# facebookresearch/FBTT-Embedding

Measured on AMD Instinct MI355X. Metric: fwd+bwd GFLOPS (true algorithmic: 3 x fwd FLOP / time), TT-EmbeddingBag E=11M D=64 ranks=[32, 32] nnz=10240, higher is better.
Workload: dtype f32

## Files before the change

fbtt-embedding_amd/csrc/ttx_internal.h:

```cpp
#pragma once
#include <hip/hip_runtime.h>
#include <stdint.h>
#include <stdio.h>
#include <string.h>

#include "../../include/ttx.h"
#ifdef TTX_TEST_HOOKS
#include "../../include/ttx_test_hooks.h"
#define TTX_KNOB(type, name, dflt) type name = dflt
#else
#define TTX_KNOB(type, name, dflt) constexpr type name = dflt
#endif

namespace ttx {

constexpr int kWave = 64;

void set_error(const char* fmt, ...);
#define TTX_FAIL(code, ...)     \
  do {                          \
    ttx::set_error(__VA_ARGS__); \
    return (code);              \
  } while (0)
#define TTX_HIP(call)                                                         \
  do {                                                                        \
    hipError_t e__ = (call);                                                  \
    if (e__ != hipSuccess)                                                    \
      TTX_FAIL(TTX_EHIP, "%s failed: %s", #call, hipGetErrorString(e__));     \
  } while (0)

inline size_t align_up(size_t x, size_t a = 256) { return (x + a - 1) / a * a; }

int allow_dynamic_lds(const void* kernel, int bytes);
int device_cus();

struct UDiv {
  unsigned m, sh1, sh2, d;
};

struct TabGeom {
  int p[TTX_MAX_TABLES_MIXED][TTX_MAX_CORES];
  int base[TTX_MAX_TABLES_MIXED][TTX_MAX_CORES];
  long long L[TTX_MAX_TABLES_MIXED][TTX_MAX_CORES];
};

struct Dims {
  int T, num_tables;
  const TabGeom* tab;
  int p[TTX_MAX_CORES], q[TTX_MAX_CORES], r[TTX_MAX_CORES + 1];
  long long L[TTX_MAX_CORES];
  int slice[TTX_MAX_CORES];
  int S[TTX_MAX_CORES];
  int m[TTX_MAX_CORES], k[TTX_MAX_CORES], n[TTX_MAX_CORES];
  int D;
  int idx32;
  UDiv dvL[TTX_MAX_CORES], dvP[TTX_MAX_CORES];
};

int make_dims(const ttx_geom* g, Dims* d);

#ifndef TTX_SEG_THIN
#define TTX_SEG_THIN 256
#endif
#ifndef TTX_HOT_PIVOT
#define TTX_HOT_PIVOT 16
#endif
constexpr int kSegThin = TTX_SEG_THIN;
constexpr int kHotRowsPivot = TTX_HOT_PIVOT;

constexpr int kHdrT4Valid = 20;
struct Plan {
  int* hdr;
  int* sid[TTX_MAX_CORES];
  int* perm[TTX_MAX_CORES];
  int* ipos[TTX_MAX_CORES];
  int* off[TTX_MAX_CORES];
  int* chunk_off;
  int4* chunk_rec;
  int4* lrec;
  int* lrow;
  int* cnt;
  int* scratch[TTX_MAX_CORES][3];
  int max_chunks;
  int MC;
  float* t4m;
  float* t4g;
  int4* t4o;
};

int choose_chunk(const Dims& d, long long nnz);
size_t t4_scratch_floats(const Dims& d);
int max_chunks(const Dims& d, long long nnz, int MC);
size_t plan_bytes(const Dims& d, long long nnz);
Plan carve_plan(const Dims& d, long long nnz, void* base);
int plan_build(const Dims& d, long long nnz, const int64_t* indices,
               const int64_t* tableidx, const int64_t* rowidx, const Plan& P, hipStream_t stream,
               const int* n_dev = nullptr, const int64_t* offsets = nullptr, int bags_per_table = 0);

constexpr int kMaxMulti = 16;
struct ProBatch {
  const int64_t* indices[kMaxMulti];
  const int64_t* offsets[kMaxMulti];
  long long out_stride;
  long long plan_stride;
};
#define TTX_PICK_BATCH(MB, Z, IND, OFF)                                                                   \
  switch (Z) {                                                                                            \
    case 1: IND = MB.indices[1]; OFF = MB.offsets[1]; break;                                              \
    case 2: IND = MB.indices[2]; OFF = MB.offsets[2]; break;                                              \
    case 3: IND = MB.indices[3]; OFF = MB.offsets[3]; break;                                              \
    case 4: IND = MB.indices[4]; OFF = MB.offsets[4]; break;                                              \
    case 5: IND = MB.indices[5]; OFF = MB.offsets[5]; break;                                              \
    case 6: IND = MB.indices[6]; OFF = MB.offsets[6]; break;                                              \
    case 7: IND = MB.indices[7]; OFF = MB.offsets[7]; break;                                              \
    case 8: IND = MB.indices[8]; OFF = MB.offsets[8]; break;                                              \
    case 9: IND = MB.indices[9]; OFF = MB.offsets[9]; break;                                              \
    case 10: IND = MB.indices[10]; OFF = MB.offsets[10]; break;                                           \
    case 11: IND = MB.indices[11]; OFF = MB.offsets[11]; break;                                           \
    case 12: IND = MB.indices[12]; OFF = MB.offsets[12]; break;                                           \
    case 13: IND = MB.indices[13]; OFF = MB.offsets[13]; break;                                           \
    case 14: IND = MB.indices[14]; OFF = MB.offsets[14]; break;                                           \
    case 15: IND = MB.indices[15]; OFF = MB.offsets[15]; break;                                           \
    default: break;                                                                                       \
  }
bool plan_batches_ok(const Dims& d, long long nnz);
int plan_build_batches(const Dims& d, int nbatch, long long nnz, const int* n_dev, const int64_t* indices,
                       const int64_t* tableidx, const int64_t* rowidx, void* plans, size_t plan_stride,
                       hipStream_t stream);

long long* debug_stamps();

int fill_iota64(int64_t* dst, long long n, hipStream_t stream);

struct DedupMap {
  int* nu;
  int64_t* uidx;
  int64_t* utab;
  int64_t* iota;
  int* uid;
  int* occ;
  int* occ_off;
};
constexpr int kDedupMaxN = 16384;
__host__ __device__ inline int64_t* dedup_tstart(const DedupMap& M) { return (int64_t*)((char*)M.nu + 64); }
int dedup_max_tables();
bool plan_groups_tables(const Dims& d, long long N);
bool dedup_supported(const Dims& d, long long nnz);
size_t dedup_bytes(long long nnz);
DedupMap carve_dedup(long long nnz, void* base);
int dedup_build(const Dims& d, long long nnz, const int64_t* indices, const int64_t* tableidx, const DedupMap& M,
                hipStream_t stream);
void dedup_key_buffers(const DedupMap& M, long long nnz, int64_t** keys, int64_t** vals);
int dedup_build_from_keys(long long nnz, unsigned long long all, const DedupMap& M, hipStream_t stream);
size_t gsum_scratch_bytes(int D, long long nnz);
int gsum_launch(const DedupMap& M, long long nnz, int B, int D, const int64_t* rowidx, const int64_t* tableidx, const float* psw,
                const float* d_output, float* Gu, void* scratch, hipStream_t st, long long skip_key = -1);

size_t sort_pairs_ws_bytes(int64_t n);
int sort_pairs_desc(int64_t n, const int64_t* keys_in, const int64_t* vals_in, char* ws, int64_t** keys_sorted,
                    int64_t** vals_sorted, hipStream_t st, int passes);

size_t populate_sort_ws_bytes(int64_t H);
int populate_sort_mark(int64_t H, int64_t* hashtbl, int64_t* cache_freq, int32_t* cache_state, int64_t cache_size,
                       int keep_state, char* ws, int64_t** sorted_keys, hipStream_t st);

void prof_begin(int which, hipStream_t s);
void prof_end(int which, hipStream_t s);
struct ProfScope {
  int w;
  hipStream_t s;
  ProfScope(int which, hipStream_t st) : w(which), s(st) { prof_begin(w, s); }
// ... 91 lines not shown
```

fbtt-embedding_amd/csrc/ttx_plan.hip:

```cpp
#include <stdlib.h>

#include <type_traits>

#include "ttx_internal.h"

namespace ttx {

constexpr int kPlanThreads = 1024;
constexpr int kPlanWaves = kPlanThreads / kWave;

#ifdef TTX_TEST_HOOKS
static int g_plan_route = 0;
#define TTX_PLAN_ROUTE(id) (g_plan_route = (id))
#else
#define TTX_PLAN_ROUTE(id) ((void)0)
#endif

int max_chunks(const Dims& d, long long nnz, int MC) {
  if (MC <= 0) MC = 1;
  long long a = nnz < d.S[1] ? nnz : d.S[1];
  long long v = a + nnz / MC + 1;
  return (int)v;
}

static size_t r64(size_t k) { return (k + 63) / 64 * 64; }

constexpr int kMaxGroupsHost = 32;
static size_t cnt_ints(const Dims& d, long long nnz) {
  return (size_t)d.T * (256 * ((nnz + 255) / 256 + 1) + 2048 * (kMaxGroupsHost + 2));
}

static size_t plan_ints(const Dims& d, long long nnz, int MC) {
  size_t n = r64(64);
  for (int t = 0; t < d.T; ++t) n += r64(nnz) * 6 + r64((size_t)d.S[t] + 1);
  n += r64((size_t)d.S[1] + 1);
  n += r64((size_t)max_chunks(d, nnz, MC) * 4);
  n += r64((size_t)nnz * 4);
  n += r64((size_t)nnz);
  n += r64(cnt_ints(d, nnz));
  if (const size_t tf = t4_scratch_floats(d)) n += 2 * r64((size_t)nnz * tf) + r64((size_t)nnz * 4);
  return n;
}

size_t plan_bytes(const Dims& d, long long nnz) {
  return align_up(plan_ints(d, nnz, choose_chunk(d, nnz)) * sizeof(int));
}

Plan carve_plan(const Dims& d, long long nnz, void* base) {
  Plan P;
  memset(&P, 0, sizeof(P));
  P.MC = choose_chunk(d, nnz);
  P.max_chunks = max_chunks(d, nnz, P.MC);
  int* cur = (int*)base;
  auto take = [&](size_t k) { int* r = cur; cur += r64(k); return r; };
  P.hdr = take(64);
  P.chunk_rec = (int4*)take((size_t)P.max_chunks * 4);
  P.lrec = (int4*)take((size_t)nnz * 4);
  P.lrow = take(nnz);
  P.cnt = take(cnt_ints(d, nnz));
  for (int t = 0; t < d.T; ++t) {
    P.sid[t] = take(nnz);
    P.perm[t] = take(nnz);
    P.ipos[t] = take(nnz);
    P.off[t] = take((size_t)d.S[t] + 1);
    for (int i = 0; i < 3; ++i) P.scratch[t][i] = take(nnz);
  }
  P.chunk_off = take((size_t)d.S[1] + 1);
  if (const size_t tf = t4_scratch_floats(d)) {
    P.t4m = (float*)take((size_t)nnz * tf);
    P.t4g = (float*)take((size_t)nnz * tf);
    P.t4o = (int4*)take((size_t)nnz * 4);
  }
  return P;
}

__device__ __forceinline__ int block_excl_scan(int v, int* wtot, int* total) {
  const int lane = lane_id();
  const int w = threadIdx.x / kWave;
  int inc = wave_incl_scan(v);
  if (lane == kWave - 1) wtot[w] = inc;
  __syncthreads();
  if (threadIdx.x == 0) {
    int run = 0;
    for (int i = 0; i < kPlanWaves; ++i) { int c = wtot[i]; wtot[i] = run; run += c; }
    wtot[kPlanWaves] = run;
  }
  __syncthreads();
  int res = wtot[w] + inc - v;
  *total = wtot[kPlanWaves];
  __syncthreads();
  return res;
}

struct CoreDec {
  UDiv dl, dp;
  long long L;
  int p, first, idx32;
};
__device__ __forceinline__ CoreDec core_dec(const Dims& d, int t) {
  CoreDec c;
  c.dl = d.dvL[t];
  c.dp = d.dvP[t];
  c.L = d.L[t];
  c.p = d.p[t];
  c.first = (t == 0);
  c.idx32 = d.idx32;
  return c;
}
__device__ __forceinline__ int decode_core(const CoreDec& c, long long idx) {
  if (idx < 0) idx = 0;
  if (c.idx32 && (unsigned long long)idx < (1ull << 32)) {
    const unsigned q = udiv((unsigned)idx, c.dl);
    const unsigned a = c.first ? q : q - udiv(q, c.dp) * c.dp.d;
    return (int)min(a, (unsigned)(c.p - 1));
  }
  long long a = idx / c.L;
  if (!c.first) a = a % c.p;
  if (a >= c.p) a = c.p - 1;
  return (int)a;
}
__device__ __forceinline__ int decode_core(const Dims& d, int t, long long idx) {
  return decode_core(core_dec(d, t), idx);
}
__device__ __forceinline__ int slice_id(const Dims& d, const CoreDec& ct, int t, int tb, long long idx) {
  if (!d.tab) return tb * ct.p + decode_core(ct, idx);
  tb = min(max(tb, 0), d.num_tables - 1);
  const int p = d.tab->p[tb][t];
  const long long L = d.tab->L[tb][t];
  if (idx < 0) idx = 0;
  long long a;
  if ((((unsigned long long)idx | (unsigned long long)L) >> 32) == 0) a = (unsigned)idx / (unsigned)L;
  else a = idx / L;
  if (t > 0) a %= p;
  if (a >= p) a = p - 1;
  return d.tab->base[tb][t] + (int)a;
// ... 192 lines not shown
    if (tid == 0) {
      P.chunk_off[S1] = carry;
      P.hdr[0] = carry;
      P.hdr[1] = MC;
      P.hdr[2] = N;
      P.hdr[3] = rowidx ? 1 : 0;
      P.hdr[kHdrT4Valid] = 0;
      for (int tt = 0; tt < TTX_MAX_CORES; ++tt) P.hdr[8 + tt] = -1;
    }
    PSTAMP(5);
  }
#undef PSTAMP
}

constexpr int kMbThreads = 256;
constexpr int kMbUnits = kMbThreads / kWave;
constexpr int kSB = 4;
constexpr int kMbFuseU = 256;

struct MbArgs {
  int N, U;
  const int* n_dev;
  int unit;
  int* cnt;
};

__device__ __forceinline__ int live_n(int n_host, const int* n_dev) {
  if (!n_dev) return n_host;
  const int v = *n_dev;
  return v < 0 ? 0 : (v < n_host ? v : n_host);
}

struct MbItem { int val, kv; };

__device__ __forceinline__ MbItem mb_load(int i, bool valid, int pass, const Dims& d, int t, const CoreDec& ct,
                                          const int64_t* __restrict__ indices, const int64_t* __restrict__ tableidx,
                                          const int* __restrict__ src, const int* __restrict__ key) {
  MbItem it{0, 0};
  if (!valid) return it;
  if (pass == 0) {
    const int tb = tableidx ? (int)tableidx[i] : 0;
    it.val = i;
    it.kv = slice_id(d, ct, t, tb, indices[i]);
  } else {
    it.val = src[i];
    it.kv = key[it.val];
  }
  return it;
}

__global__ __launch_bounds__(kMbThreads) void mb_count_kernel(
    Dims d, MbArgs A, const int64_t* __restrict__ indices, const int64_t* __restrict__ tableidx) {
  __shared__ int hist[kMbUnits][256];
  const int t = blockIdx.y;
  const int lane = lane_id(), w = threadIdx.x / kWave;
  const int u = blockIdx.x * kMbUnits + w;
  for (int e = lane; e < 256; e += kWave) hist[w][e] = 0;
  const int N = live_n(A.N, A.n_dev);
  const int beg = min(N, u * A.unit), end = min(N, beg + A.unit);
  const CoreDec ct = core_dec(d, t);
  for (int base = beg; base < end; base += kSB * kWave) {
    MbItem it[kSB];
#pragma unroll
    for (int k = 0; k < kSB; ++k) {
      const int i = base + k * kWave + lane;
      it[k] = mb_load(i, i < end, 0, d, t, ct, indices, tableidx, nullptr, nullptr);
    }
#pragma unroll
    for (int k = 0; k < kSB; ++k) {
      const int i = base + k * kWave + lane;
      const bool valid = i < end;
      const unsigned dg = (unsigned)it[k].kv & 255u;
      const unsigned long long peers = wave_match8(dg, valid);
      if (valid && (peers & lanemask_lt()) == 0) hist[w][dg] += __popcll(peers);
    }
  }
  if (u < A.U)
    for (int e = lane; e < 256; e += kWave) A.cnt[((size_t)t * A.U + u) * 256 + e] = hist[w][e];
}

template <typename T>
__device__ __forceinline__ T* shifted(T* p, long long bytes) { return (T*)((char*)p + bytes); }

__device__ __forceinline__ void finish_single_pass(const Dims& d, int t, int dg, int tot, int dbase, int N,
                                                   bool has_row, const Plan& P, int* wt5, long long psh = 0) {
  int* const hdr = (int*)((char*)P.hdr + psh);
  int* const chunk_off = (int*)((char*)P.chunk_off + psh);
  int4* const chunk_rec = (int4*)((char*)P.chunk_rec + psh);
  const int lane = lane_id(), w = threadIdx.x / kWave;
  const int S = d.S[t];
  if (t != 1) {
    const int nhot = __syncthreads_count(dg < S && tot > 2 * kSegThin);
    if (dg == 0) hdr[8 + t] = nhot;
    if (dg <= S) shifted(P.off[t], psh)[dg] = (dg == S) ? N : dbase;
    if (dg == 0 && S == 256) shifted(P.off[t], psh)[256] = N;
    return;
  }
  const int MC = P.MC;
  const int nf = dg < S ? tot / MC : 0;
  const int pr = dg < S ? tot - nf * MC : 0;
  const int np = pr ? 1 : 0;
  const int nhot = __syncthreads_count(nf + np > kHotRowsPivot);
  if (dg == 0) hdr[8 + 1] = nhot;
  const int packed = (nf << 12) | np;
  const int cinc = wave_incl_scan(packed);
  __syncthreads();
  if (lane == kWave - 1 && w < kMbUnits) wt5[w] = cinc;
  __syncthreads();
  int cb = 0, call = 0;
  for (int k = 0; k < kMbUnits; ++k) { const int v = wt5[k]; if (k < w) cb += v; call += v; }
  const int exq = cb + cinc - packed;
  const int fbase = exq >> 12, pbase = exq & 4095;
  const int ftot = call >> 12, ptot = call & 4095;
  const int ctot = ftot + ptot;
  const int ex = fbase + pbase;
  __shared__ int cf_base[257], cf_pos[256], cf_slot[256];
  if (dg < S) {
    chunk_off[dg] = ex;
    cf_base[dg] = fbase;
    cf_pos[dg] = dbase;
    cf_slot[dg] = ex;
    if (np) chunk_rec[ftot + pbase] = make_int4(dg, dbase + nf * MC, pr, ex + nf);
  }
  if (dg == 0) cf_base[S] = ftot;
  __syncthreads();
  for (int c = threadIdx.x; c < ftot; c += blockDim.x) {
    int lo = 0, hi = S;
    while (hi - lo > 1) {
      const int mid = (lo + hi) >> 1;
      if (cf_base[mid] <= c) lo = mid; else hi = mid;
    }
    const int j = c - cf_base[lo];
    chunk_rec[c] = make_int4(lo, cf_pos[lo] + j * MC, MC, cf_slot[lo] + j);
  }
  for (int cc = ctot + dg; cc < P.max_chunks; cc += blockDim.x) chunk_rec[cc] = make_int4(0, 0, 0, 0);
  if (dg == 0) {
    chunk_off[S] = ctot;
    hdr[0] = ctot;
    hdr[1] = MC;
    hdr[2] = N;
    hdr[3] = has_row ? 1 : 0;
    hdr[kHdrT4Valid] = 0;
  }
}

constexpr int kOneUnit = 64;
constexpr int kOneMaxN = 16384;
constexpr int kProMaxBags = 4096;
struct Prologue {
  const int64_t* offsets;
  int nb;
  int64_t* rowidx;
  int64_t* tableidx;
  int H;
  int64_t* hashtbl;
  int64_t* cache_freq;
};
#ifndef TTX_PLAN_XWG
#define TTX_PLAN_XWG 1
#endif
constexpr int kOneThreads = 1024;
constexpr int kOneWaves = kOneThreads / kWave;
template <bool PRO>
__global__ __launch_bounds__(kOneThreads) void mb_single_kernel(
    Dims d, int Nmax, const int* __restrict__ n_dev, const int64_t* __restrict__ indices,
    const int64_t* __restrict__ tableidx, const int64_t* __restrict__ rowidx, Plan P, Prologue pg, ProBatch mb) {
  if (PRO && blockIdx.z > 0) {
    const int z = blockIdx.z;
    TTX_PICK_BATCH(mb, z, indices, pg.offsets)
    pg.rowidx += (long long)z * mb.out_stride;
    pg.tableidx += (long long)z * mb.out_stride;
  }
  if (!PRO && blockIdx.z > 0) {
    const long long sh = (long long)blockIdx.z * mb.out_stride;
    indices += sh;
    if (tableidx) tableidx += sh;
    if (rowidx) rowidx += sh;
    if (n_dev) n_dev += blockIdx.z;
  }
  const long long psh = (long long)blockIdx.z * mb.plan_stride;
  __shared__ int haft[256], hbef[256], hrun[kOneWaves][256];
  const int N = live_n(Nmax, n_dev);
  __shared__ int wt5[kMbUnits + 1];
  __shared__ int offs[PRO ? kProMaxBags + 1 : 1];
  const int t = blockIdx.y, tid = threadIdx.x;
  const int lane = lane_id(), w = tid / kWave;
  const CoreDec ct = core_dec(d, t);
  if (PRO) tableidx = nullptr;
  constexpr int kMaxB = kOneMaxN / kOneThreads;
  const int nbat = (N + kOneThreads - 1) / kOneThreads;
  long long ix[kMaxB];
  int tb[kMaxB];
#pragma unroll
  for (int m = 0; m < kMaxB; ++m) {
    const int i = m * kOneThreads + tid;
    ix[m] = (m < nbat && i < N) ? indices[i] : 0;
    tb[m] = (m < nbat && i < N && tableidx) ? (int)tableidx[i] : 0;
  }
  if (PRO) {
    if (t <= 1)
      for (int e = tid; e <= pg.nb; e += kOneThreads) offs[e] = (int)min(pg.offsets[e], (int64_t)0x7fffffff);
  }
  if (tid < 256) { haft[tid] = 0; hbef[tid] = 0; }
  for (int e = tid; e < kOneWaves * 256; e += kOneThreads) (&hrun[0][0])[e] = 0;
  __syncthreads();
  const int bx = blockIdx.x;
  const int bbeg = bx * (kOneWaves * kOneUnit), bend = min(N, bbeg + kOneWaves * kOneUnit);
  const int i = bbeg + tid;
  const bool valid = i < bend;
  int kv = 0, tbv = 0, row = 0;
  long long idx = 0;
  bool peel_on = true;
#pragma unroll
  for (int m = 0; m < kMaxB; ++m) {
    if (m < nbat) {
      const int im = m * kOneThreads + tid;
// ... 204 lines not shown
      a += len > 0 ? (len + kWideSpan - 1) / kWideSpan : 1;
    }
    gwg[ga.ngroups] = a;
  }
  __syncthreads();
  const int g = blockIdx.x;
  if (g >= gwg[ga.ngroups]) return false;
  int k = 0;
  while (k + 1 < ga.ngroups && gwg[k + 1] <= g) ++k;
  m->k = k;
  m->tb0 = k * ga.gsz;
  m->pos0 = gpos[k];
  m->beg = min(gpos[k + 1], gpos[k] + (g - gwg[k]) * kWideSpan);
  m->end = min(gpos[k + 1], m->beg + kWideSpan);
  m->wg0 = gwg[k];
  m->wg1 = gwg[k + 1];
  return true;
}
__device__ __forceinline__ int slice_base(const Dims& d, const CoreDec& ct, int t, int tb) {
  if (tb >= d.num_tables) return d.S[t];
  return d.tab ? d.tab->base[tb][t] : tb * ct.p;
}

template <int BITS, bool GRP>
__global__ __launch_bounds__(kWideThreads) void mbw_count_kernel(
    Dims d, int Nmax, const int* __restrict__ n_dev, const int64_t* __restrict__ indices,
    const int64_t* __restrict__ tableidx, int* __restrict__ cnt, GrpArgs ga) {
  constexpr int BINS = 1 << BITS;
  __shared__ int hist[BINS];
  __shared__ int gpos[GRP ? kMaxGroups + 1 : 1], gwg[GRP ? kMaxGroups + 1 : 1];
  const int t = blockIdx.y, tid = threadIdx.x;
  for (int e = tid; e < BINS; e += kWideThreads) hist[e] = 0;
  const int N = live_n(Nmax, n_dev);
  const CoreDec ct = core_dec(d, t);
  int beg = blockIdx.x * kWideSpan, end = min(N, beg + kWideSpan), sb = 0;
  if (GRP) {
    GrpMap m;
    if (!grp_map(d, ga, N, gpos, gwg, &m)) return;
    beg = m.beg;
    end = m.end;
    sb = slice_base(d, ct, t, m.tb0);
  } else {
    __syncthreads();
  }
  long long ix[kSB];
  int tb[kSB];
#pragma unroll
  for (int k = 0; k < kSB; ++k) {
    const int i = beg + k * kWideThreads + tid;
    ix[k] = i < end ? indices[i] : 0;
    tb[k] = (i < end && tableidx) ? (int)tableidx[i] : 0;
  }
#pragma unroll
  for (int k = 0; k < kSB; ++k) {
    const int i = beg + k * kWideThreads + tid;
    if (i < end) atomicAdd(&hist[min(max(slice_id(d, ct, t, tb[k], ix[k]) - sb, 0), BINS - 1)], 1);
  }
  __syncthreads();
  int* row = cnt + ((size_t)t * gridDim.x + blockIdx.x) * BINS;
  for (int e = tid; e < BINS; e += kWideThreads) row[e] = hist[e];
}

template <int K>
__device__ __forceinline__ void finish_wide(const Dims& d, int t, const int (&tot)[K], const int (&dbase)[K], int N,
                                            bool has_row, const Plan& P, int* wt) {
  const int tid = threadIdx.x, lane = lane_id(), w = tid / kWave;
  const int S = d.S[t];
  if (t != 1) {
    int nh = 0;
#pragma unroll
    for (int j = 0; j < K; ++j) {
      const int dg = tid * K + j;
      if (dg < S) P.off[t][dg] = dbase[j];
      nh += (dg < S && tot[j] > 2 * kSegThin) ? 1 : 0;
    }
    if (tid == 0) wt[0] = 0;
    __syncthreads();
    if (nh) atomicAdd(&wt[0], nh);
    __syncthreads();
    if (tid == 0) { P.off[t][S] = N; P.hdr[8 + t] = wt[0]; }
    return;
  }
  const int MC = P.MC;
  int nf[K], pr[K], packed[K], psum = 0;
#pragma unroll
  for (int j = 0; j < K; ++j) {
    const int dg = tid * K + j;
    nf[j] = dg < S ? tot[j] / MC : 0;
    pr[j] = dg < S ? tot[j] - nf[j] * MC : 0;
    packed[j] = (nf[j] << 13) | (pr[j] ? 1 : 0);
    psum += packed[j];
  }
  const int cinc = wave_incl_scan(psum);
  __syncthreads();
  if (lane == kWave - 1) wt[w] = cinc;
  __syncthreads();
  int cb = 0, call = 0;
  for (int k = 0; k < kWideWaves; ++k) { const int v = wt[k]; if (k < w) cb += v; call += v; }
  int exq = cb + cinc - psum;
  const int ftot = call >> 13, ptot = call & 8191;
  const int ctot = ftot + ptot;
#pragma unroll
  for (int j = 0; j < K; ++j) {
    const int dg = tid * K + j;
    const int fbase = exq >> 13, pbase = exq & 8191;
    const int ex = fbase + pbase;
    if (dg < S) {
      P.chunk_off[dg] = ex;
      for (int jj = 0; jj < nf[j]; ++jj) P.chunk_rec[fbase + jj] = make_int4(dg, dbase[j] + jj * MC, MC, ex + jj);
      if (pr[j]) P.chunk_rec[ftot + pbase] = make_int4(dg, dbase[j] + nf[j] * MC, pr[j], ex + nf[j]);
    }
    exq += packed[j];
  }
  for (int cc = ctot + tid; cc < P.max_chunks; cc += kWideThreads) P.chunk_rec[cc] = make_int4(0, 0, 0, 0);
  int nh = 0;
#pragma unroll
  for (int j = 0; j < K; ++j) nh += (tid * K + j < S && nf[j] + (pr[j] ? 1 : 0) > kHotRowsPivot) ? 1 : 0;
  __syncthreads();
  if (tid == 0) wt[0] = 0;
  __syncthreads();
  if (nh) atomicAdd(&wt[0], nh);
  __syncthreads();
  if (tid == 0) {
    P.chunk_off[S] = ctot;
    P.hdr[0] = ctot;
    P.hdr[1] = MC;
    P.hdr[2] = N;
    P.hdr[3] = has_row ? 1 : 0;
    P.hdr[kHdrT4Valid] = 0;
    P.hdr[8 + 1] = wt[0] ? -1 : 0;
  }
}

template <int BITS, bool GRP>
__global__ __launch_bounds__(kWideThreads) void mbw_scatter_kernel(
    Dims d, int Nmax, const int* __restrict__ n_dev, const int64_t* __restrict__ indices,
    const int64_t* __restrict__ tableidx, const int64_t* __restrict__ rowidx, const int* __restrict__ cnt, Plan P,
    GrpArgs ga) {
  constexpr int BINS = 1 << BITS, K = BINS / kWideThreads;
  constexpr bool REL = BITS >= 12;
  using Cnt = typename std::conditional<REL, unsigned short, int>::type;
  extern __shared__ int wide_lds[];
  Cnt (*hrun)[BINS] = (Cnt (*)[BINS])wide_lds;
  int* wt = wide_lds + kWideWaves * BINS * (int)sizeof(Cnt) / (int)sizeof(int);
  int* hbase = wt + kWideWaves;
  __shared__ int gpos[GRP ? kMaxGroups + 1 : 1], gwg[GRP ? kMaxGroups + 1 : 1];
  const int t = blockIdx.y, tid = threadIdx.x, lane = lane_id(), w = tid / kWave;
  const int N = live_n(Nmax, n_dev);
  const CoreDec ct = core_dec(d, t);
  int beg = blockIdx.x * kWideSpan, end = min(N, beg + kWideSpan), sb = 0, pos0 = 0, wg0 = 0, wg1 = gridDim.x;
  int grp = 0, sg = d.S[t];
  if (GRP) {
    GrpMap m;
    if (!grp_map(d, ga, N, gpos, gwg, &m)) return;
    beg = m.beg; end = m.end; pos0 = m.pos0; wg0 = m.wg0; wg1 = m.wg1; grp = m.k;
    sb = slice_base(d, ct, t, m.tb0);
    sg = slice_base(d, ct, t, m.tb0 + ga.gsz) - sb;
  }
  {
    int4* z = (int4*)&hrun[w][0];
    constexpr int kRowVec = BINS * (int)sizeof(Cnt) / 16;
    for (int e = lane; e < kRowVec; e += kWave) z[e] = make_int4(0, 0, 0, 0);
  }
  long long ix[kSB];
  int tb[kSB], kv[kSB], brow[kSB];
  unsigned long long peers[kSB];
  const int wbeg = beg + w * (kSB * kWave);
#pragma unroll
  for (int k = 0; k < kSB; ++k) {
    const int i = wbeg + k * kWave + lane;
    ix[k] = i < end ? indices[i] : 0;
    tb[k] = (i < end && tableidx) ? (int)tableidx[i] : 0;
    brow[k] = (t == 1 && rowidx && i < end) ? (int)rowidx[i] : 0;
  }
  int tot[K], bef[K], dbase[K], sum = 0;
#pragma unroll
  for (int j = 0; j < K; ++j) { tot[j] = 0; bef[j] = 0; }
  {
    const int* c = cnt + (size_t)t * gridDim.x * BINS + tid * K;
    for (int g0 = wg0; g0 < wg1; g0 += 8) {
      int v[8][K];
#pragma unroll
      for (int r = 0; r < 8; ++r)
#pragma unroll
        for (int j = 0; j < K; ++j) v[r][j] = (g0 + r < wg1) ? c[(size_t)(g0 + r) * BINS + j] : 0;
#pragma unroll
      for (int r = 0; r < 8; ++r)
#pragma unroll
        for (int j = 0; j < K; ++j) {
          tot[j] += v[r][j];
          if (g0 + r < (int)blockIdx.x) bef[j] += v[r][j];
        }
    }
  }
#pragma unroll
// ... 1029 lines not shown
```

fbtt-embedding_amd/csrc/ttx_tt.hip:

```cpp
#include "ttx_tt_common.h"

namespace ttx {

#include "ttx_tt_generic.inc"

__global__ __launch_bounds__(kThreads) void pool_kernel(int Nmax, const int* __restrict__ hdr, int B, int D,
                                                       const int64_t* __restrict__ rowidx,
                                                       const int64_t* __restrict__ tableidx,
                                                       const float* __restrict__ rows,
                                                       const float* __restrict__ psw, float* __restrict__ out) {
  const int n = blockIdx.x * (kThreads / 32) + threadIdx.x / 32;
  const int l = threadIdx.x & 31;
  const int N = min(Nmax, hdr[2]);
  if (n >= N) return;
  const int64_t r = rowidx[n], tb = tableidx[n];
  if (n > 0 && rowidx[n - 1] == r && tableidx[n - 1] == tb) return;
  const unsigned long long half = (threadIdx.x & 32) ? 0xffffffff00000000ull : 0x00000000ffffffffull;
  int sl = 1;
  for (;;) {
    const int c = n + sl + l;
    const bool same = c < N && rowidx[c] == r && tableidx[c] == tb;
    unsigned long long m = (__ballot(!same) & half) >> (threadIdx.x & 32);
    if (m) { sl += __builtin_ctzll(m); break; }
    sl += 32;
// ... 1769 lines not shown
}

static int run_bwd_spec(TTX_SPEC_BWD_ARGS) {
  int rc = spec_bwd_32(id, d, P, C, B, rowidx, d_output, PC, pad, R, st);
  if (rc == kSpecNotMine) rc = spec_bwd_64(id, d, P, C, B, rowidx, d_output, PC, pad, R, st);
  if (rc == kSpecNotMine) rc = spec_bwd_16(id, d, P, C, B, rowidx, d_output, PC, pad, R, st);
  if (rc == kSpecNotMine) rc = spec_bwd_128a(id, d, P, C, B, rowidx, d_output, PC, pad, R, st);
  if (rc == kSpecNotMine) rc = spec_bwd_128b(id, d, P, C, B, rowidx, d_output, PC, pad, R, st);
  if (rc == kSpecNotMine) rc = spec_bwd_128c(id, d, P, C, B, rowidx, d_output, PC, pad, R, st);
  if (rc == kSpecNotMine) TTX_FAIL(TTX_EUNSUPPORTED, "no specialised backward kernel");
  return rc;
}

static int run_rows(const Dims& d, long long nnz, const Plan& P, const float* const* cores,
                    float* rows, float* zout, long long nzero, hipStream_t st, const PoolFuse* fuse = nullptr,
                    bool* fused = nullptr) {
  if (fused) *fused = false;
  bool pad = false;
  Dims d3;
  if (t4_merge_dims(d, &d3)) {
    if (!P.t4m) TTX_FAIL(TTX_EINVAL, "internal: the plan carries no scratch for the four-core route");
    const SpecId id = spec_match(d3, &pad);
    ProfScope ps(TTX_PROF_FWD, st);
    const int rcm = t4_merge(d, nnz, P, cores[2], cores[3], st, 0);
    if (rcm) return rcm;
    CorePtrs C;
    for (int t = 0; t < TTX_MAX_CORES; ++t) C.c[t] = nullptr;
    C.c[0] = (float*)cores[0]; C.c[1] = (float*)cores[1]; C.c[2] = P.t4m;
    RealDims R = real_dims(d3);
    R.c2n = 1;
    bool did = false;
    const PoolFuse none{};
    return run_rows_spec(id, P, C, rows, zout, nzero, none, &did, pad, R, st);
  }
  if (t2_shape(d)) {
    const T2Lds L = t2_lds(d, false);
    CorePtrs C;
    for (int t = 0; t < TTX_MAX_CORES; ++t) C.c[t] = t < d.T ? (float*)cores[t] : nullptr;
    ProfScope ps(TTX_PROF_FWD, st);
    hipLaunchKernelGGL(t2_fwd_kernel, dim3(P.max_chunks), dim3(kT2Threads), L.floats * sizeof(float), st, d, P, C, rows, zout,
                       nzero, L);
    TTX_HIP(hipGetLastError());
    return TTX_OK;
  }
  if (const SpecId id = spec_match(d, &pad)) {
    CorePtrs C;
    for (int t = 0; t < TTX_MAX_CORES; ++t) C.c[t] = t < d.T ? (float*)cores[t] : nullptr;
    ProfScope ps(TTX_PROF_FWD, st);
    bool did = fuse != nullptr && fuse->arrive != nullptr && !pad;
    const PoolFuse none{};
    const int rc = run_rows_spec(id, P, C, rows, zout, nzero, fuse ? *fuse : none, &did, pad, real_dims(d), st);
    if (fused) *fused = did;
    return rc;
  }
  Lds L;
  int rc = generic_lds(d, P, false, &L);
  if (rc) return rc;
  rc = allow_lds(fwd_kernel, L.bytes);
  if (rc) return rc;
  CorePtrs C;
  for (int t = 0; t < TTX_MAX_CORES; ++t) C.c[t] = t < d.T ? (float*)cores[t] : nullptr;
  ProfScope ps(TTX_PROF_FWD, st);
  hipLaunchKernelGGL(fwd_kernel, dim3(P.max_chunks), dim3(kThreads), L.bytes, st, d, P, C, rows, L, zout, nzero);
  TTX_HIP(hipGetLastError());
  return TTX_OK;
}

}

using namespace ttx;

extern "C" {

#ifdef TTX_TEST_HOOKS
int ttx_debug_stamps(void* device_buffer) {
  g_stamps = (long long*)device_buffer;
  return TTX_OK;
}

int ttx_debug_skip(int32_t mask) {
  g_disable_spec = (mask & 256) ? 1 : 0;
  g_disable_pad = (mask & 32768) ? 1 : 0;
  g_no_pack = (mask >> 16) & 1;
  g_skip_launch = (mask >> 9) & 63;
  mask &= 255;
  g_debug_skip = mask;
  return TTX_OK;
}

int ttx_debug_lds_budget(int32_t bytes) {
  if (bytes < 0 || bytes > 160 * 1024) TTX_FAIL(TTX_EINVAL, "LDS budget %d out of range", bytes);
  g_lds_budget = bytes ? bytes : 160 * 1024;
  return TTX_OK;
}

int ttx_set_chunk(int32_t mc) {
  if (mc < 0 || mc > 64) TTX_FAIL(TTX_EINVAL, "chunk %d out of range 0..64", mc);
  g_chunk_override = mc;
  return TTX_OK;
}
#endif

int ttx_debug_tiles(const ttx_geom* g, int32_t* out) {
  Dims d;
  int rc = make_dims(g, &d);
  if (rc) return rc;
  if (!out) TTX_FAIL(TTX_EINVAL, "out is NULL");
  for (int i = 0; i < 6; ++i) out[i] = 0;
  if (spec_shape(d) || t4_merge_dims(d, nullptr) || t2_shape(d)) return TTX_OK;
  const TileCfg cfg = choose_tiles(d);
  if (cfg.MC <= 0) return TTX_OK;
  const Lds L = make_lds(d, cfg.MC, true, cfg.bpp, cfg.KB);
  out[0] = L.MC; out[1] = L.bpp; out[2] = L.KB; out[3] = L.ncp; out[4] = L.nkb; out[5] = L.bytes;
  return TTX_OK;
}

int ttx_debug_state(void) {
  return ((g_debug_skip | g_skip_launch | g_disable_spec | g_disable_pad | g_no_pack) ? 1 : 0) | (g_lds_budget != 160 * 1024 ? 2 : 0) |
         (g_chunk_override ? 4 : 0) | (g_stamps ? 8 : 0) | (ttx_cache_debug_state() << 4);
}

int ttx_has_test_hooks(void) {
#ifdef TTX_TEST_HOOKS
  return 1;
#else
  return 0;
#endif
}

size_t ttx_tt_forward_workspace_bytes(const ttx_geom* g, int32_t B, int32_t D, int64_t nnz) {
  (void)B; (void)D;
  Dims d;
  if (make_dims(g, &d) != TTX_OK || nnz < 0) return 0;
  return plan_bytes(d, nnz) + rows_bytes(d, nnz) + 256;
}

static int common_checks(const Dims& d, int32_t D, int64_t nnz) {
  if (D <= 0) TTX_FAIL(TTX_EINVAL, "D=%d must be > 0", D);
  if (D != d.D) TTX_FAIL(TTX_EINVAL, "D=%d does not match prod(q)=%d", D, d.D);
  if (nnz < 0 || nnz >= (1ll << 31)) TTX_FAIL(TTX_EINVAL, "nnz=%lld out of range", (long long)nnz);
  if (choose_chunk(d, nnz) <= 0)
    TTX_FAIL(TTX_EUNSUPPORTED, "no tiling of this TT shape fits the LDS (one q1 block of x_0 is %d x %d floats per lookup)",
             d.q[0], d.T >= 3 ? d.k[1] : d.n[0]);
  return TTX_OK;
}

int ttx_tt_forward(const ttx_geom* g, int32_t B, int32_t D, int64_t nnz, const int64_t* indices,
                   const int64_t* rowidx, const int64_t* tableidx, const float* const* tt_cores,
                   float* output, const void* plan, void* workspace, size_t workspace_bytes,
                   ttx_stream_t stream) {
  return ttx_tt_forward_w(g, B, D, nnz, indices, rowidx, tableidx, nullptr, tt_cores, output, plan, workspace,
                          workspace_bytes, stream);
}

int ttx_tt_forward_w(const ttx_geom* g, int32_t B, int32_t D, int64_t nnz, const int64_t* indices,
                     const int64_t* rowidx, const int64_t* tableidx, const float* psw,
                     const float* const* tt_cores, float* output, const void* plan, void* workspace,
                     size_t workspace_bytes, ttx_stream_t stream) {
  return ttx_tt_forward_wr(g, B, D, nnz, indices, rowidx, tableidx, psw, tt_cores, output, nullptr, plan, workspace,
                           workspace_bytes, stream);
}

int ttx_tt_forward_wr(const ttx_geom* g, int32_t B, int32_t D, int64_t nnz, const int64_t* indices,
                      const int64_t* rowidx, const int64_t* tableidx, const float* psw,
                      const float* const* tt_cores, float* output, float* rows_keep, const void* plan, void* workspace,
                      size_t workspace_bytes, ttx_stream_t stream) {
  return ttx_tt_forward_o(g, B, D, nnz, indices, rowidx, tableidx, psw, tt_cores, output, rows_keep, nullptr, nullptr, plan,
                          workspace, workspace_bytes, stream);
}

int64_t ttx_tt_forward_arrive_ints(const ttx_geom* g, int64_t nnz) {
  Dims d;
  bool pad = false;
  if (make_dims(g, &d) != TTX_OK || nnz <= 0 || nnz > kPoolSpanMin || d.D % 4 != 0 || !spec_match(d, &pad) || pad) return 0;
  return nnz;
}

static int tt_forward_impl(const ttx_geom* g, int32_t B, int32_t D, int64_t nnz, const int64_t* indices,
                           const int64_t* rowidx, const int64_t* tableidx, const float* psw,
                           const float* const* tt_cores, float* output, float* rows_keep, const int64_t* offsets,
                           int32_t* arrive, const void* plan, void* workspace, size_t workspace_bytes, ttx_stream_t stream,
                           const int32_t* cache_loc, const float* cache_weight);

int ttx_tt_forward_o(const ttx_geom* g, int32_t B, int32_t D, int64_t nnz, const int64_t* indices,
                     const int64_t* rowidx, const int64_t* tableidx, const float* psw,
                     const float* const* tt_cores, float* output, float* rows_keep, const int64_t* offsets,
                     int32_t* arrive, const void* plan, void* workspace, size_t workspace_bytes, ttx_stream_t stream) {
  return tt_forward_impl(g, B, D, nnz, indices, rowidx, tableidx, psw, tt_cores, output, rows_keep, offsets, arrive, plan, workspace,
                         workspace_bytes, stream, nullptr, nullptr);
}

int ttx_tt_forward_cached_supported(const ttx_geom* g, int32_t D, int64_t nnz) {
  static const bool off = getenv("TTX_NO_FUSED_CACHE_GATHER") != nullptr;
  return !off && g && g->num_tables == 1 && nnz > 0 && nnz <= kPoolSpanMin && D % 4 == 0 && D / 4 <= 4 * kThreads;
}

int ttx_tt_forward_cached(const ttx_geom* g, int32_t B, int32_t D, int64_t nnz, const int64_t* indices,
                          const int64_t* rowidx, const int64_t* tableidx, const float* const* tt_cores,
                          const int32_t* cache_loc, const float* cache_weight, float* output, const void* plan,
                          void* workspace, size_t workspace_bytes, ttx_stream_t stream) {
  if (!ttx_tt_forward_cached_supported(g, D, nnz)) TTX_FAIL(TTX_EUNSUPPORTED, "ttx_tt_forward_cached: not for this call");
// ... 557 lines not shown
```

Before: 27900.

## Interleave chunk records into column-major dispatch order across eight columns

Chunk records are no longer laid out as all full chunks followed by the partial ones. They are now written in the natural per-row order and then permuted into an eight-column interleaved layout. Consecutive dispatched chunks therefore come from different rows spread across the table, which is meant to balance work and reduce contention on the same rows among concurrently running blocks. The cost is extra index arithmetic in plan building and less locality between adjacent workgroups.

```diff
diff --git a/fbtt-embedding_amd/csrc/ttx_internal.h b/fbtt-embedding_amd/csrc/ttx_internal.h
--- a/fbtt-embedding_amd/csrc/ttx_internal.h
+++ b/fbtt-embedding_amd/csrc/ttx_internal.h
@@ -86,7 +86,15 @@
   float* t4m;
   float* t4g;
   int4* t4o;
-};
+  int cols;
+};
+
+constexpr int kChunkCols = 8;
+#ifdef TTX_TEST_HOOKS
+extern int g_chunk_cols;
+#else
+constexpr int g_chunk_cols = kChunkCols;
+#endif
 
 int choose_chunk(const Dims& d, long long nnz);
 size_t t4_scratch_floats(const Dims& d);
diff --git a/fbtt-embedding_amd/csrc/ttx_plan.hip b/fbtt-embedding_amd/csrc/ttx_plan.hip
--- a/fbtt-embedding_amd/csrc/ttx_plan.hip
+++ b/fbtt-embedding_amd/csrc/ttx_plan.hip
@@ -12,6 +12,7 @@
 #ifdef TTX_TEST_HOOKS
 static int g_plan_route = 0;
 #define TTX_PLAN_ROUTE(id) (g_plan_route = (id))
+int g_chunk_cols = kChunkCols;
 #else
 #define TTX_PLAN_ROUTE(id) ((void)0)
 #endif
@@ -51,6 +52,7 @@
   memset(&P, 0, sizeof(P));
   P.MC = choose_chunk(d, nnz);
   P.max_chunks = max_chunks(d, nnz, P.MC);
+  P.cols = g_chunk_cols;
   int* cur = (int*)base;
   auto take = [&](size_t k) { int* r = cur; cur += r64(k); return r; };
   P.hdr = take(64);
@@ -409,6 +411,28 @@
 template <typename T>
 __device__ __forceinline__ T* shifted(T* p, long long bytes) { return (T*)((char*)p + bytes); }
 
+struct ChunkCols { int C, K, rem, head; };
+__device__ __forceinline__ ChunkCols chunk_cols(int n, int C) {
+  const int K = n / C, rem = n - K * C;
+  return ChunkCols{C, K, rem, rem * (K + 1)};
+}
+__device__ __forceinline__ int chunk_dispatch_index(const ChunkCols& cc, int x) {
+  if (x < cc.head) return cc.C * (x % (cc.K + 1)) + x / (cc.K + 1);
+  const int y = x - cc.head;
+  return cc.C * (y % cc.K) + cc.rem + y / cc.K;
+}
+struct ChunkWalk { int r, k; };
+__device__ __forceinline__ ChunkWalk chunk_walk(const ChunkCols& cc, int x) {
+  if (x < cc.head) return ChunkWalk{x / (cc.K + 1), x % (cc.K + 1)};
+  const int y = x - cc.head;
+  return ChunkWalk{cc.rem + y / cc.K, y % cc.K};
+}
+__device__ __forceinline__ int chunk_walk_next(const ChunkCols& cc, ChunkWalk& w) {
+  const int idx = cc.C * w.k + w.r;
+  if (++w.k == cc.K + (w.r < cc.rem ? 1 : 0)) { w.k = 0; ++w.r; }
+  return idx;
+}
+
 __device__ __forceinline__ void finish_single_pass(const Dims& d, int t, int dg, int tot, int dbase, int N,
                                                    bool has_row, const Plan& P, int* wt5, long long psh = 0) {
   int* const hdr = (int*)((char*)P.hdr + psh);
@@ -425,40 +449,34 @@
   }
   const int MC = P.MC;
   const int nf = dg < S ? tot / MC : 0;
-  const int pr = dg < S ? tot - nf * MC : 0;
-  const int np = pr ? 1 : 0;
+  const int np = (dg < S && tot > nf * MC) ? 1 : 0;
+  const int nch = nf + np;
   const int nhot = __syncthreads_count(nf + np > kHotRowsPivot);
   if (dg == 0) hdr[8 + 1] = nhot;
-  const int packed = (nf << 12) | np;
-  const int cinc = wave_incl_scan(packed);
+  const int cinc = wave_incl_scan(nch);
   __syncthreads();
   if (lane == kWave - 1 && w < kMbUnits) wt5[w] = cinc;
   __syncthreads();
-  int cb = 0, call = 0;
-  for (int k = 0; k < kMbUnits; ++k) { const int v = wt5[k]; if (k < w) cb += v; call += v; }
-  const int exq = cb + cinc - packed;
-  const int fbase = exq >> 12, pbase = exq & 4095;
-  const int ftot = call >> 12, ptot = call & 4095;
-  const int ctot = ftot + ptot;
-  const int ex = fbase + pbase;
-  __shared__ int cf_base[257], cf_pos[256], cf_slot[256];
+  int cb = 0, ctot = 0;
+  for (int k = 0; k < kMbUnits; ++k) { const int v = wt5[k]; if (k < w) cb += v; ctot += v; }
+  const int ex = cb + cinc - nch;
+  __shared__ int cf_slot[256], cf_pos[256], cf_tot[256];
   if (dg < S) {
     chunk_off[dg] = ex;
-    cf_base[dg] = fbase;
+    cf_slot[dg] = ex;
     cf_pos[dg] = dbase;
-    cf_slot[dg] = ex;
-    if (np) chunk_rec[ftot + pbase] = make_int4(dg, dbase + nf * MC, pr, ex + nf);
-  }
-  if (dg == 0) cf_base[S] = ftot;
-  __syncthreads();
-  for (int c = threadIdx.x; c < ftot; c += blockDim.x) {
+    cf_tot[dg] = tot;
+  }
+  __syncthreads();
+  const ChunkCols cols = chunk_cols(ctot, P.cols);
+  for (int c = threadIdx.x; c < ctot; c += blockDim.x) {
     int lo = 0, hi = S;
     while (hi - lo > 1) {
       const int mid = (lo + hi) >> 1;
-      if (cf_base[mid] <= c) lo = mid; else hi = mid;
-    }
-    const int j = c - cf_base[lo];
-    chunk_rec[c] = make_int4(lo, cf_pos[lo] + j * MC, MC, cf_slot[lo] + j);
+      if (cf_slot[mid] <= c) lo = mid; else hi = mid;
+    }
+    const int j = c - cf_slot[lo];
+    chunk_rec[chunk_dispatch_index(cols, c)] = make_int4(lo, cf_pos[lo] + j * MC, min(MC, cf_tot[lo] - j * MC), c);
   }
   for (int cc = ctot + dg; cc < P.max_chunks; cc += blockDim.x) chunk_rec[cc] = make_int4(0, 0, 0, 0);
   if (dg == 0) {
@@ -829,35 +847,35 @@
     return;
   }
   const int MC = P.MC;
-  int nf[K], pr[K], packed[K], psum = 0;
+  int nf[K], pr[K], psum = 0;
 #pragma unroll
   for (int j = 0; j < K; ++j) {
     const int dg = tid * K + j;
     nf[j] = dg < S ? tot[j] / MC : 0;
     pr[j] = dg < S ? tot[j] - nf[j] * MC : 0;
-    packed[j] = (nf[j] << 13) | (pr[j] ? 1 : 0);
-    psum += packed[j];
+    psum += nf[j] + (pr[j] ? 1 : 0);
   }
   const int cinc = wave_incl_scan(psum);
   __syncthreads();
   if (lane == kWave - 1) wt[w] = cinc;
   __syncthreads();
-  int cb = 0, call = 0;
-  for (int k = 0; k < kWideWaves; ++k) { const int v = wt[k]; if (k < w) cb += v; call += v; }
-  int exq = cb + cinc - psum;
-  const int ftot = call >> 13, ptot = call & 8191;
-  const int ctot = ftot + ptot;
+  int cb = 0, ctot = 0;
+  for (int k = 0; k < kWideWaves; ++k) { const int v = wt[k]; if (k < w) cb += v; ctot += v; }
+  int ex = cb + cinc - psum;
+  const ChunkCols cols = chunk_cols(ctot, P.cols);
 #pragma unroll
   for (int j = 0; j < K; ++j) {
     const int dg = tid * K + j;
-    const int fbase = exq >> 13, pbase = exq & 8191;
-    const int ex = fbase + pbase;
     if (dg < S) {
       P.chunk_off[dg] = ex;
-      for (int jj = 0; jj < nf[j]; ++jj) P.chunk_rec[fbase + jj] = make_int4(dg, dbase[j] + jj * MC, MC, ex + jj);
-      if (pr[j]) P.chunk_rec[ftot + pbase] = make_int4(dg, dbase[j] + nf[j] * MC, pr[j], ex + nf[j]);
-    }
-    exq += packed[j];
+      if (nf[j] || pr[j]) {
+        ChunkWalk cw = chunk_walk(cols, ex);
+        for (int jj = 0; jj < nf[j]; ++jj)
+          P.chunk_rec[chunk_walk_next(cols, cw)] = make_int4(dg, dbase[j] + jj * MC, MC, ex + jj);
+        if (pr[j]) P.chunk_rec[chunk_walk_next(cols, cw)] = make_int4(dg, dbase[j] + nf[j] * MC, pr[j], ex + nf[j]);
+      }
+    }
+    ex += nf[j] + (pr[j] ? 1 : 0);
   }
   for (int cc = ctot + tid; cc < P.max_chunks; cc += kWideThreads) P.chunk_rec[cc] = make_int4(0, 0, 0, 0);
   int nh = 0;
diff --git a/fbtt-embedding_amd/csrc/ttx_tt.hip b/fbtt-embedding_amd/csrc/ttx_tt.hip
--- a/fbtt-embedding_amd/csrc/ttx_tt.hip
+++ b/fbtt-embedding_amd/csrc/ttx_tt.hip
@@ -1875,6 +1875,7 @@
   g_disable_spec = (mask & 256) ? 1 : 0;
   g_disable_pad = (mask & 32768) ? 1 : 0;
   g_no_pack = (mask >> 16) & 1;
+  g_chunk_cols = (mask >> 17) & 1 ? 1 : kChunkCols;
   g_skip_launch = (mask >> 9) & 63;
   mask &= 255;
   g_debug_skip = mask;
@@ -1909,7 +1910,7 @@
 }
 
 int ttx_debug_state(void) {
-  return ((g_debug_skip | g_skip_launch | g_disable_spec | g_disable_pad | g_no_pack) ? 1 : 0) | (g_lds_budget != 160 * 1024 ? 2 : 0) |
+  return ((g_debug_skip | g_skip_launch | g_disable_spec | g_disable_pad | g_no_pack | (g_chunk_cols != kChunkCols)) ? 1 : 0) | (g_lds_budget != 160 * 1024 ? 2 : 0) |
          (g_chunk_override ? 4 : 0) | (g_stamps ? 8 : 0) | (ttx_cache_debug_state() << 4);
 }
 
```

New measurement: 28540 (median of 6 runs). 2.3% higher.
